# jnbraun/bcnn

Hardware: AMD Instinct MI355X
Metric: images/sec fwd+bwd (higher is better)
Workload: dtype f32; 1 GPU; ResNet-18 224x224 (BASELINE configs[2]), N=128 per GPU, fwd+bwd+SGD through bcnn_net C API; CIFAR-example topology + ImageNet stem, fc-1000; batch_per_gpu=128, global_batch=128, parallelism=dp1, comm=none (one rank)

## Files before the change

### bcnn_amd/csrc/conv_dw_dma.hip

```cpp
#include "conv_paths.h"
#include "lds_dma.h"

namespace bcnn_hip {

struct DwDmaArgs {
    const float* x;
    const float* dy;
    float* partials;
    ConvShape s;
    int mtiles, ntiles;
    int qsplits, q_per_split;
    int Mpad, Npad;
    unsigned x_bytes, dy_bytes;
    unsigned ow_magic;
    int b_row_stride;
    int kk2;
    int rowmode, nrows, row_kk, row_ks, row_plane, row_pitch;
    unsigned row_kk_magic, row_ks_magic;
};

constexpr int DWQ = 32;
constexpr int DWPAIR = 66;

template <int WM, int WN, int WTM, int WTN>
__global__ __launch_bounds__(64 * WM * WN) void conv_dw_dma_kernel(const DwDmaArgs a) {
    constexpr int NW = WM * WN;
    constexpr int BM = 32 * WM * WTM, BN = 32 * WN * WTN;
    static_assert((BM / 2) % NW == 0 && (BN / 2) % NW == 0, "row pairs must split evenly over the waves");
    constexpr int APAIRS = BM / 2, BPAIRS = BN / 2;
    constexpr int BUF = (APAIRS + BPAIRS) * DWPAIR;
    __shared__ float lds[2 * BUF];

    const ConvShape& s = a.s;
    const int tid = threadIdx.x, lane = tid & 63;
    const int wid = __builtin_amdgcn_readfirstlane(tid >> 6);
    const int wm = wid / WN, wn = wid % WN;
    const int l31 = lane & 31, lhi = lane >> 5;
    const int g = blockIdx.y;
    const int lb = xcd_remap(blockIdx.x, gridDim.x);
    const int tap = lb % a.kk2;
    const int rest = lb / a.kk2;
    const int tiles = a.mtiles * a.ntiles;
    const int tile = rest % tiles, qs = rest / tiles;
    const int mt = tile % a.mtiles, nt = tile / a.mtiles;
    const int f0 = mt * BM, c0 = nt * BN;
    const int kr = s.pointwise ? 0 : tap / s.ksz, kc = s.pointwise ? 0 : tap - (tap / s.ksz) * s.ksz;

    const unsigned qbeg = (unsigned)qs * (unsigned)a.q_per_split;
    unsigned qend = qbeg + (unsigned)a.q_per_split;
    if (qend > (unsigned)s.total_q) qend = (unsigned)s.total_q;
    const int nkt = qbeg < qend ? (int)((qend - qbeg + DWQ - 1) / DWQ) : 0;

    unsigned q = qbeg + (unsigned)l31;
    unsigned n = q / (unsigned)s.OHOW;
    unsigned pix = q - n * (unsigned)s.OHOW;
    const unsigned row_a = (unsigned)lhi * (unsigned)s.OHOW, row_b = a.rowmode ? 0u : (unsigned)lhi * (unsigned)a.b_row_stride;
    unsigned va = kOOB, vb = kOOB;
    auto lane_offsets = [&]() {
        const bool qv = q < qend;
        const unsigned offa = n * (unsigned)(s.F * s.OHOW) + pix + row_a;
        unsigned offb;
        bool ok = qv;
        if (s.pointwise) {
            offb = n * (unsigned)(s.C * s.HW) + pix + row_b;
        } else {
            const unsigned oh = magic_div(pix, a.ow_magic), ow = pix - oh * (unsigned)s.OW;
            const int ih = (int)oh * s.stride - s.pad + kr, iw = (int)ow * s.stride - s.pad + kc;
            ok = ok && (unsigned)ih < (unsigned)s.H && (unsigned)iw < (unsigned)s.W;
            offb = (n * (unsigned)(s.C * s.H) + (unsigned)ih) * (unsigned)s.W + (unsigned)iw + row_b;
        }
        va = qv ? offa * 4u : kOOB;
        vb = ok ? offb * 4u : kOOB;
    };
    auto advance = [&]() {
        q += DWQ; pix += DWQ;
        if (pix >= (unsigned)s.OHOW) { pix -= (unsigned)s.OHOW; ++n; }
    };

    const rsrc_i4 rs_a = make_rsrc(a.dy, a.dy_bytes), rs_b = make_rsrc(a.x, a.x_bytes);
    const unsigned lds0 = lds_offset(&lds[0]);
    const unsigned a_row0 = (unsigned)(g * s.Mg), b_grp = (unsigned)(g * s.Cg) * (unsigned)s.HW;

    auto stage = [&](int buf) {
        const unsigned base = lds0 + (unsigned)(buf * BUF * 4);
#pragma unroll
        for (int i = 0; i < APAIRS / NW; ++i) {
            const int p = wid * (APAIRS / NW) + i;
            const int f = f0 + 2 * p;
            const unsigned soff = (a_row0 + (unsigned)(f < s.Mg ? f : 0)) * (unsigned)s.OHOW * 4u;
            dma_row(rs_a, base + (unsigned)(p * DWPAIR * 4), va, soff);
        }
#pragma unroll
        for (int i = 0; i < BPAIRS / NW; ++i) {
            const int p = wid * (BPAIRS / NW) + i;
            const int c = c0 + 2 * p;
            if (a.rowmode) {
                auto row_off = [&](int j) -> unsigned {
                    if (j >= a.nrows) j = 0;
                    const unsigned ch = magic_div((unsigned)j, a.row_kk_magic), r = (unsigned)j - ch * (unsigned)a.row_kk;
                    const unsigned kr = magic_div(r, a.row_ks_magic), kc = r - kr * (unsigned)a.row_ks;
                    return (ch * (unsigned)a.row_plane + kr * (unsigned)a.row_pitch + kc) * 4u;
                };
                const unsigned o0 = row_off(c), o1 = row_off(c + 1);
                const unsigned vbp = vb == kOOB ? kOOB : vb + (unsigned)lhi * (o1 - o0);
                dma_row(rs_b, base + (unsigned)((APAIRS + p) * DWPAIR * 4), vbp, o0);
            } else {
                const unsigned soff = (b_grp + (unsigned)(c < s.Cg ? c : 0) * (unsigned)a.b_row_stride) * 4u;
                dma_row(rs_b, base + (unsigned)((APAIRS + p) * DWPAIR * 4), vb, soff);
            }
        }
    };

    f32x16 acc[WTM][WTN];
#pragma unroll
    for (int i = 0; i < WTM; ++i)
#pragma unroll
        for (int j = 0; j < WTN; ++j)
#pragma unroll
            for (int r = 0; r < 16; ++r) acc[i][j][r] = 0.f;

    int a_off[WTM], b_off[WTN];
#pragma unroll
    for (int i = 0; i < WTM; ++i) a_off[i] = ((wm * WTM + i) * 16 + (l31 >> 1)) * DWPAIR + (l31 & 1) * 32 + 2 * lhi;
#pragma unroll
    for (int j = 0; j < WTN; ++j) b_off[j] = (APAIRS + (wn * WTN + j) * 16 + (l31 >> 1)) * DWPAIR + (l31 & 1) * 32 + 2 * lhi;

    if (nkt > 0) {
        lane_offsets();
        stage(0);
    }
    dma_wait();
    __syncthreads();
    for (int it = 0; it < nkt; ++it) {
        const int cur = it & 1;
        if (it + 1 < nkt) {
            advance();
            lane_offsets();
            stage(cur ^ 1);
        }
        const float* buf = lds + cur * BUF;
#pragma unroll
        for (int kp = 0; kp < DWQ / 4; ++kp) {
            float2 av[WTM], bv[WTN];
#pragma unroll
            for (int i = 0; i < WTM; ++i) av[i] = *reinterpret_cast<const float2*>(buf + a_off[i] + 4 * kp);
#pragma unroll
            for (int j = 0; j < WTN; ++j) bv[j] = *reinterpret_cast<const float2*>(buf + b_off[j] + 4 * kp);
#pragma unroll
            for (int i = 0; i < WTM; ++i)
#pragma unroll
                for (int j = 0; j < WTN; ++j) acc[i][j] = mfma32(av[i].x, bv[j].x, acc[i][j]);
#pragma unroll
            for (int i = 0; i < WTM; ++i)
#pragma unroll
                for (int j = 0; j < WTN; ++j) acc[i][j] = mfma32(av[i].y, bv[j].y, acc[i][j]);
        }
        dma_wait();
        __syncthreads();
    }

    float* out = a.partials + ((((size_t)qs * s.groups + g) * a.kk2 + tap) * a.Mpad) * (size_t)a.Npad;
#pragma unroll
    for (int i = 0; i < WTM; ++i)
#pragma unroll
        for (int j = 0; j < WTN; ++j) {
            float v[16];
#pragma unroll
            for (int r = 0; r < 16; ++r) v[r] = acc[i][j][r];
#pragma unroll
            for (int r = 0; r < 16; ++r) {
                const int f = f0 + (wm * WTM + i) * 32 + mfma_row(r, lane);
                const int c = c0 + (wn * WTN + j) * 32 + l31;
                out[(size_t)f * a.Npad + c] = v[r];
            }
        }
}

template <int NSUB>
__global__ __launch_bounds__(64 * NSUB) void conv_dw_dma_finalize_kernel(const float* __restrict__ partials,
                                                                        int qsplits, int groups, int Mg, int Cg,
                                                                        int kk2, int Mpad, int Npad,
                                                                        float* __restrict__ dw,
                                                                        const float* __restrict__ fold_var,
                                                                        const float* __restrict__ fold_scales) {
    __shared__ float red[NSUB][64];
    const int tx = threadIdx.x & 63, ty = threadIdx.x >> 6;
    const size_t total = (size_t)groups * kk2 * Mg * Cg;
    const size_t i = (size_t)blockIdx.x * 64 + tx;
    const size_t plane = (size_t)Mpad * Npad;
    const size_t qstride = (size_t)groups * kk2 * plane;
    float sum = 0.f;
    size_t o = 0;
    if (i < total) {
        const int c = (int)(i % Cg);
        size_t t = i / Cg;
        const int f = (int)(t % Mg);
        t /= Mg;
        const int tap = (int)(t % kk2), g = (int)(t / kk2);
        const float* p = partials + ((size_t)g * kk2 + tap) * plane + (size_t)f * Npad + c;
        int qs = ty;
        float s0 = 0.f, s1 = 0.f, s2 = 0.f, s3 = 0.f;
        for (; qs + 3 * NSUB < qsplits; qs += 4 * NSUB) {
            const float v0 = p[(size_t)qs * qstride], v1 = p[(size_t)(qs + NSUB) * qstride];
            const float v2 = p[(size_t)(qs + 2 * NSUB) * qstride], v3 = p[(size_t)(qs + 3 * NSUB) * qstride];
            s0 += v0; s1 += v1; s2 += v2; s3 += v3;
        }
        for (; qs < qsplits; qs += NSUB) s0 += p[(size_t)qs * qstride];
        sum = (s0 + s1) + (s2 + s3);
        o = (((size_t)g * Mg + f) * Cg + c) * kk2 + tap;
    }
    red[ty][tx] = sum;
    __syncthreads();
    if (ty == 0 && i < total) {
        float tot = 0.f;
#pragma unroll
        for (int r = 0; r < NSUB; ++r) tot += red[r][tx];
        if (fold_var) tot *= bnfold_a(fold_var, fold_scales, (int)((i / ((size_t)Mg * Cg * kk2)) * Cg + (i % Cg)));
        dw[o] += tot;
    }
}

template <int NSUB>
__global__ __launch_bounds__(64 * NSUB) void conv_dw_dma_finalize_x4_kernel(const float* __restrict__ partials, int qsplits,
                                                                           int groups, int Mg, int Cg, int Mpad, int Npad,
                                                                           float* __restrict__ dw,
                                                                           const float* __restrict__ fold_var,
                                                                           const float* __restrict__ fold_scales) {
    __shared__ float4 red[NSUB][64];
    const int tx = threadIdx.x & 63, ty = threadIdx.x >> 6;
    const size_t total4 = (size_t)groups * Mg * Cg / 4;
    const size_t i4 = (size_t)blockIdx.x * 64 + tx;
    const size_t plane = (size_t)Mpad * Npad;
    const size_t qstride = (size_t)groups * plane;
    float4 sum = make_float4(0.f, 0.f, 0.f, 0.f);
    if (i4 < total4) {
        const size_t i = i4 * 4;
        const int c = (int)(i % Cg);
        const size_t t = i / Cg;
        const int f = (int)(t % Mg), g = (int)(t / Mg);
        const float* p = partials + (size_t)g * plane + (size_t)f * Npad + c;
        auto ld = [&](int qs) { return *reinterpret_cast<const float4*>(p + (size_t)qs * qstride); };
        auto acc = [](float4& a, const float4& v) { a.x += v.x; a.y += v.y; a.z += v.z; a.w += v.w; };
        float4 s0 = sum, s1 = sum, s2 = sum, s3 = sum;
        int qs = ty;
        for (; qs + 3 * NSUB < qsplits; qs += 4 * NSUB) {
            const float4 v0 = ld(qs), v1 = ld(qs + NSUB), v2 = ld(qs + 2 * NSUB), v3 = ld(qs + 3 * NSUB);
            acc(s0, v0); acc(s1, v1); acc(s2, v2); acc(s3, v3);
        }
        for (; qs < qsplits; qs += NSUB) acc(s0, ld(qs));
        sum = make_float4((s0.x + s1.x) + (s2.x + s3.x), (s0.y + s1.y) + (s2.y + s3.y), (s0.z + s1.z) + (s2.z + s3.z),
                          (s0.w + s1.w) + (s2.w + s3.w));
    }
    red[ty][tx] = sum;
    __syncthreads();
    if (ty == 0 && i4 < total4) {
        float4 tot = make_float4(0.f, 0.f, 0.f, 0.f);
#pragma unroll
        for (int r = 0; r < NSUB; ++r) { tot.x += red[r][tx].x; tot.y += red[r][tx].y; tot.z += red[r][tx].z; tot.w += red[r][tx].w; }
        float4* o = reinterpret_cast<float4*>(dw) + i4;
        if (fold_var) {
            const size_t i = i4 * 4;
            const int c = (int)(i % Cg) + (int)(i / ((size_t)Mg * Cg)) * Cg;
            tot.x *= bnfold_a(fold_var, fold_scales, c); tot.y *= bnfold_a(fold_var, fold_scales, c + 1);
            tot.z *= bnfold_a(fold_var, fold_scales, c + 2); tot.w *= bnfold_a(fold_var, fold_scales, c + 3);
        }
        float4 d = *o;
        d.x += tot.x; d.y += tot.y; d.z += tot.z; d.w += tot.w;
        *o = d;
    }
}

struct DwTile { int bm, bn, threads; };
constexpr int kNumDwTiles = 6;
static const DwTile kDwTiles[kNumDwTiles] = {
    {64, 64, 256},
    {128, 64, 256},
    {128, 64, 512},
    {128, 128, 256},
    {128, 128, 1024},
    {64, 128, 512},
};

struct DwDmaPlan {
    bool ok;
    int cfg;
    int mtiles, ntiles, qsplits, q_per_split, Mpad, Npad, kk2;
    size_t partial_floats;
};

static DwDmaPlan plan_dw_dma(const ConvShape& s) {
    DwDmaPlan p;
    p.ok = false;
    p.partial_floats = 0;
    if (s.ksz > 7 && !s.pointwise) return p;
    if (s.Mg < 32 || s.Cg < 16 || (s.Mg & 1) || (s.Cg & 1)) return p;
    if (s.OHOW < DWQ || s.total_q < 4 * DWQ) return p;
    if ((size_t)s.N * s.C * s.HW * 4 >= 0x7ffffff0ull || (size_t)s.N * s.F * s.OHOW * 4 >= 0x7ffffff0ull) return p;
    p.kk2 = s.pointwise ? 1 : s.ksz * s.ksz;
    p.cfg = s.Mg > 64 ? 1 : 0;
    static const char* forced = BCNN_EXP_ENV("BCNN_HIP_DW_TILE");
    if (forced && forced[0] >= '0' && forced[0] < '0' + kNumDwTiles) p.cfg = forced[0] - '0';
    static const char* wantenv = BCNN_EXP_ENV("BCNN_HIP_DW_WANT");
    const int want_per_cu = wantenv ? atoi(wantenv) : 8;
    const int BM = kDwTiles[p.cfg].bm, BN = kDwTiles[p.cfg].bn;
    p.mtiles = ceil_div(s.Mg, BM); p.ntiles = ceil_div(s.Cg, BN);
    p.Mpad = p.mtiles * BM; p.Npad = p.ntiles * BN;
    const long long tiles = (long long)p.mtiles * p.ntiles * p.kk2 * s.groups;
    long long want = ((long long)want_per_cu * kCUs + tiles - 1) / tiles;
    const long long maxs = (s.total_q + 8 * DWQ - 1) / (8 * DWQ);
    if (want > maxs) want = maxs;
    if (want < 1) want = 1;
    long long per = (s.total_q + want - 1) / want;
    per = (per + DWQ - 1) / DWQ * DWQ;
    p.q_per_split = (int)per;
    p.qsplits = (int)((s.total_q + per - 1) / per);
    p.partial_floats = (size_t)p.qsplits * s.groups * p.kk2 * (size_t)p.Mpad * p.Npad;
    p.ok = true;
    return p;
}

size_t conv_dw_dma_workspace_floats(const ConvShape& s) { return plan_dw_dma(s).partial_floats; }


bool conv_backward_weights_dma(const float* x, const float* dy, float* dw, const ConvShape& s, float* workspace,
                               size_t workspace_floats, const BnFold* fold) {
    const DwDmaPlan p = plan_dw_dma(s);
    if (!p.ok) return false;
    conv_require_workspace(workspace, workspace_floats, p.partial_floats);
    DwDmaArgs a;
    a.rowmode = 0; a.nrows = 0;
    a.x = x; a.dy = dy; a.partials = workspace; a.s = s;
    a.mtiles = p.mtiles; a.ntiles = p.ntiles; a.qsplits = p.qsplits; a.q_per_split = p.q_per_split;
    a.Mpad = p.Mpad; a.Npad = p.Npad; a.kk2 = p.kk2;
    a.x_bytes = (unsigned)((size_t)s.N * s.C * s.HW * 4);
    a.dy_bytes = (unsigned)((size_t)s.N * s.F * s.OHOW * 4);
    a.ow_magic = magic_of(s.OW);
    a.b_row_stride = s.pointwise ? s.OHOW : s.HW;
    dim3 grid((unsigned)(p.mtiles * p.ntiles * p.kk2 * p.qsplits), (unsigned)s.groups);
    const unsigned threads = (unsigned)kDwTiles[p.cfg].threads;
    trace_kernel("conv_dw_dma_kernel");
    switch (p.cfg) {
        case 0: conv_dw_dma_kernel<2, 2, 1, 1><<<grid, threads, 0, current_stream()>>>(a); break;
        case 1: conv_dw_dma_kernel<2, 2, 2, 1><<<grid, threads, 0, current_stream()>>>(a); break;
        case 2: conv_dw_dma_kernel<4, 2, 1, 1><<<grid, threads, 0, current_stream()>>>(a); break;
        case 3: conv_dw_dma_kernel<2, 2, 2, 2><<<grid, threads, 0, current_stream()>>>(a); break;
        case 4: conv_dw_dma_kernel<4, 4, 1, 1><<<grid, threads, 0, current_stream()>>>(a); break;
        default: conv_dw_dma_kernel<2, 4, 1, 1><<<grid, threads, 0, current_stream()>>>(a); break;
    }
    KERNEL_CHECK();
    const size_t total = (size_t)s.groups * s.Mg * s.Cg * p.kk2;
    static const bool x4_on = BCNN_EXP_ENV("BCNN_HIP_NO_DW_FINALIZE_X4") == nullptr;
    if (x4_on && p.kk2 == 1 && p.qsplits > 16 && (s.Cg & 3) == 0 && (p.Npad & 3) == 0 &&
        ((reinterpret_cast<uintptr_t>(dw) | reinterpret_cast<uintptr_t>(workspace)) & 15) == 0)
        conv_dw_dma_finalize_x4_kernel<16><<<(unsigned)((total / 4 + 63) / 64), 1024, 0, current_stream()>>>(
            workspace, p.qsplits, s.groups, s.Mg, s.Cg, p.Mpad, p.Npad, dw, fold ? fold->var : nullptr, fold ? fold->scales : nullptr);
    else if (p.qsplits > 16)
        conv_dw_dma_finalize_kernel<16><<<(unsigned)((total + 63) / 64), 1024, 0, current_stream()>>>(
            workspace, p.qsplits, s.groups, s.Mg, s.Cg, p.kk2, p.Mpad, p.Npad, dw, fold ? fold->var : nullptr, fold ? fold->scales : nullptr);
    else
        conv_dw_dma_finalize_kernel<4><<<(unsigned)((total + 63) / 64), 256, 0, current_stream()>>>(
            workspace, p.qsplits, s.groups, s.Mg, s.Cg, p.kk2, p.Mpad, p.Npad, dw, fold ? fold->var : nullptr, fold ? fold->scales : nullptr);
    KERNEL_CHECK();
    return true;
}

bool conv_backward_weights_dma_timed(const float* x, const float* dy, float* dw, float*, const ConvShape& s, float* workspace,
                                     size_t workspace_floats, bool*) {
    if (!plan_dw_dma(s).ok) return false;
    KTimer kt(K_CONV_DW, conv_gemm_flops(s), conv_gemm_bytes(s));
    return conv_backward_weights_dma(x, dy, dw, s, workspace, workspace_floats, nullptr);
}


static DwDmaPlan plan_dw_small_c(const ConvShape& s) {
    DwDmaPlan p;
    p.ok = false; p.partial_floats = 0;
    if (!conv_small_c_fwd_wanted(s) || (s.Mg & 1) || s.OHOW < DWQ || s.total_q < 4 * DWQ) return p;
    p.kk2 = 1;
    p.cfg = 0;
    const int BM = kDwTiles[p.cfg].bm, BN = kDwTiles[p.cfg].bn;
    p.mtiles = ceil_div(s.Mg, BM); p.ntiles = ceil_div(s.K, BN);
    p.Mpad = p.mtiles * BM; p.Npad = p.ntiles * BN;
    const long long tiles = (long long)p.mtiles * p.ntiles;
    long long want = (8LL * kCUs + tiles - 1) / tiles;
    const long long maxs = (s.total_q + 8 * DWQ - 1) / (8 * DWQ);
    if (want > maxs) want = maxs;
    if (want < 1) want = 1;
    long long per = (s.total_q + want - 1) / want;
    per = (per + DWQ - 1) / DWQ * DWQ;
    p.q_per_split = (int)per;
    p.qsplits = (int)((s.total_q + per - 1) / per);
    p.partial_floats = (size_t)p.qsplits * (size_t)p.Mpad * p.Npad;
    p.ok = true;
    return p;
}

size_t conv_dw_small_c_workspace_floats(const ConvShape& s) { return plan_dw_small_c(s).partial_floats; }

bool conv_backward_weights_small_c(const float* x, const float* dy, float* dw, float*, const ConvShape& s, float* workspace,
                                   size_t workspace_floats, bool*) {
    const DwDmaPlan p = plan_dw_small_c(s);
    if (!p.ok) return false;
    conv_require_workspace(workspace, workspace_floats, p.partial_floats);
    KTimer kt(K_CONV_DW, conv_gemm_flops(s), conv_gemm_bytes(s));
    const int Hp = s.H + 2 * s.pad, Wp = s.W + 2 * s.pad;
    float* xp = conv_small_c_padded_input(x, s, 0, nullptr, 1);
    const ConvShape sp = make_conv_shape(s.N, s.C, Hp, Wp, s.F, s.ksz, s.stride, 0, 1);
    DwDmaArgs a;
    a.x = xp; a.dy = dy; a.partials = workspace; a.s = sp;
    a.mtiles = p.mtiles; a.ntiles = p.ntiles; a.qsplits = p.qsplits; a.q_per_split = p.q_per_split;
    a.Mpad = p.Mpad; a.Npad = p.Npad; a.kk2 = 1;
    a.x_bytes = (unsigned)((size_t)s.N * s.C * Hp * Wp * 4);
    a.dy_bytes = (unsigned)((size_t)s.N * s.F * s.OHOW * 4);
    a.ow_magic = magic_of(sp.OW);
    a.b_row_stride = 0;
    a.rowmode = 1; a.nrows = s.K; a.row_kk = s.ksz * s.ksz; a.row_ks = s.ksz; a.row_plane = Hp * Wp; a.row_pitch = Wp;
    a.row_kk_magic = magic_of(a.row_kk); a.row_ks_magic = magic_of(a.row_ks);
    dim3 grid((unsigned)(p.mtiles * p.ntiles * p.qsplits), 1u);
    conv_dw_dma_kernel<2, 2, 1, 1><<<grid, (unsigned)kDwTiles[0].threads, 0, current_stream()>>>(a);
    KERNEL_CHECK();
    const size_t total = (size_t)s.Mg * s.K;
    if (p.qsplits > 16)
        conv_dw_dma_finalize_kernel<16><<<(unsigned)((total + 63) / 64), 1024, 0, current_stream()>>>(
            workspace, p.qsplits, 1, s.Mg, s.K, 1, p.Mpad, p.Npad, dw, nullptr, nullptr);
    else
        conv_dw_dma_finalize_kernel<4><<<(unsigned)((total + 63) / 64), 256, 0, current_stream()>>>(
            workspace, p.qsplits, 1, s.Mg, s.K, 1, p.Mpad, p.Npad, dw, nullptr, nullptr);
    KERNEL_CHECK();
    return true;
}

}
```

### bcnn_amd/csrc/conv_winograd_fused.hip

```cpp
#include "conv_paths.h"
#include "lds_dma.h"
#include "wino43_pack.h"

namespace bcnn_hip {

constexpr int WF_BT = 64;
constexpr int WF_BF = 64;
constexpr int WF_KC = 8;
constexpr int WF_STAGE = 16 * WF_KC * (WF_BF + WF_BT);

struct WinoFusedArgs {
    const float* src;
    const float* upk;
    float* dst;
    const float* bias;
    const float* slopes;
    float* stats;
    int N, J, M, H, W, TH, TW;
    unsigned T;
    int Jpad, Mpad, mblocks, tblocks;
    int nfull;
    int nunits;
    int act, add_bias;
    unsigned src_bytes, upk_bytes, dst_bytes, stats_bytes;
// ... 460 lines not shown
    const unsigned grid = (unsigned)(nblocks < kCUs ? nblocks : kCUs);
    const int rem = nblocks % (int)grid;
    a.nfull = (rem > 0 && 2 * rem <= (int)grid && nblocks > (int)grid) ? nblocks - rem : nblocks;
    a.nunits = a.nfull + 2 * (nblocks - a.nfull);
    const bool plain = !a.add_bias && a.act == BCNN_HIP_ACT_NONE;
    a.tail_scr = nullptr; a.tail_q = 0; a.tail_units = 0; a.tail_scr_bytes = 0;
    static const int ksplit_on = BCNN_EXP_ENV("BCNN_HIP_NO_WINO_KSPLIT") ? 0 : 1;
    if (ksplit_on && plain && !parts && rem > 0 && nblocks > (int)grid) {
        const int NC = a.Jpad / WF_KC;
        const int q = (int)ceil_div((long long)rem * NC, (long long)grid);
        const double ep = 1.5, now = (a.nfull < nblocks ? 0.5 * NC : (double)NC) + ep, split = q + 2 * ep + 2.0;
        if (q >= 1 && q <= NC && split < now) {
            a.nfull = nblocks;
            a.nunits = nblocks - rem;
            a.tail_units = rem;
            a.tail_q = q;
            const size_t scr_floats = (size_t)2 * grid * 64 * 64 * 4;
            a.tail_scr = scratch(SCRATCH_WFUSED_TAIL, scr_floats);
            a.tail_scr_bytes = (unsigned)(scr_floats * sizeof(float));
        }
    }
    a.stats_bytes = a.stats ? (unsigned)((size_t)a.M * 2 * a.tblocks * 2 * sizeof(float)) : 0u;
    if (a.stats && (size_t)a.stats_bytes > stats->capacity * sizeof(float)) {
        fprintf(stderr, "[bcnn_hip] fused Winograd: statistics need %u bytes, the caller's buffer holds %zu\n",
                a.stats_bytes, stats->capacity * sizeof(float));
        abort();
    }
    if (a.stats && !plain) {
        fprintf(stderr, "[bcnn_hip] fused Winograd: output statistics are taken on the raw convolution output only\n");
        abort();
    }
    trace_kernel(dx_mode ? "wino_fused_kernel:dx" : "wino_fused_kernel:fwd");
#ifdef BCNN_HIP_EXPERIMENT
    if (parts == 2) { wino_bf16_launch<2>(a, w, s, dx_mode, grid, plain); }
    else if (parts == 3) { wino_bf16_launch<3>(a, w, s, dx_mode, grid, plain); }
    else
#endif
    if (a.stats) wino_fused_kernel<0, true><<<grid, 512, 0, current_stream()>>>(a);
    else if (plain) wino_fused_kernel<0, false><<<grid, 512, 0, current_stream()>>>(a);
    else if (a.act == BCNN_HIP_ACT_RELU) wino_fused_kernel<1, false><<<grid, 512, 0, current_stream()>>>(a);
    else wino_fused_kernel<2, false><<<grid, 512, 0, current_stream()>>>(a);
    KERNEL_CHECK();
    if (a.tail_units > 0) {
        trace_kernel("wino_tail_fixup");
        if (a.stats) wino_tail_fixup_kernel<true><<<(unsigned)(a.tail_units * 16), 256, 0, current_stream()>>>(a);
        else wino_tail_fixup_kernel<false><<<(unsigned)(a.tail_units * 16), 256, 0, current_stream()>>>(a);
        KERNEL_CHECK();
    }
    if (stats) stats->splits = a.stats ? 2 * a.tblocks : 0;
}

bool wino_fused_pack_plan(const ConvShape& s, int dx_mode, WinoPackJob* job, size_t* floats) {
    const int J = dx_mode ? s.F : s.C, M = dx_mode ? s.C : s.F;
    if (wino_bf16_parts(J) != 0) return false;
    job->w = nullptr; job->u = nullptr;
    job->F = s.F; job->C = s.C; job->dx_mode = dx_mode;
    job->Jpad = (J + WF_KC - 1) / WF_KC * WF_KC;
    job->Mpad = (M + WF_BF - 1) / WF_BF * WF_BF;
    job->blocks = (int)ceil_div((long long)job->Jpad * job->Mpad, 256);
    job->npos = 16;
    job->layout = 0;
    *floats = (size_t)16 * job->Jpad * job->Mpad;
    return true;
}

void wino_fused_pack_launch(const WinoPackJob* jobs_dev, int n, int max_blocks) {
    wino_pack_weights_multi_kernel<<<dim3((unsigned)max_blocks, (unsigned)n), 256, 0, current_stream()>>>(jobs_dev);
    KERNEL_CHECK();
}

static double wf_flops(const ConvShape& s) {
    const double T = (double)s.N * ((s.H + 1) / 2) * ((s.W + 1) / 2);
    return 2.0 * 16.0 * T * s.C * s.F;
}
static double wf_useful_flops(const ConvShape& s) { return 2.0 * 16.0 * ((double)s.N * s.H * s.W / 4.0) * s.C * s.F; }

bool conv_winograd_fused_fwd_wanted(const ConvShape& s, int) { return wino_fused_wanted(s, s.C, s.F); }
void conv_forward_winograd_fused(const ConvFwdCall& c) {
    const ConvShape& s = c.s;
    KTimer kt(K_CONV_FWD_WINO, wf_flops(s), conv_gemm_bytes(s), wf_useful_flops(s));
    wino_fused_run(c.x, c.w, c.y, s, 0, c.bias, c.slopes, c.raw ? BCNN_HIP_ACT_NONE : c.act, c.raw ? 0 : (c.bias != nullptr),
                   c.raw ? c.stats : nullptr);
}

bool conv_winograd_fused_dx_wanted(const ConvShape& s, int) { return wino_fused_wanted(s, s.F, s.C); }
void conv_backward_data_winograd_fused(const ConvDxCall& c) {
    const ConvShape& s = c.s;
    KTimer kt(K_CONV_DX_WINO, wf_flops(s), conv_gemm_bytes(s), wf_useful_flops(s));
    wino_fused_run(c.dy, c.w, c.dx, s, 1, nullptr, nullptr, BCNN_HIP_ACT_NONE, 0, nullptr);
}


constexpr int WD_KT = 8;
constexpr int WD_ROW = WD_KT;
constexpr int WD_OP = 16 * 64 * WD_ROW;


struct WinoDwArgs {
    const float* x;
    const float* dy;
    float* partials;
    int N, C, F, H, W, TH, TW;
    unsigned T, tiles_per_split;
    int fblocks, cblocks, splits;
    unsigned x_bytes, dy_bytes;
};

template <bool ODDW>
__global__ __launch_bounds__(512, 2) void wino_dw_fused_kernel(const WinoDwArgs a) {
    __shared__ __attribute__((aligned(16))) float lds[2 * 2 * WD_OP];
    const int tid = threadIdx.x, lane = tid & 63;
    const int wid = __builtin_amdgcn_readfirstlane(tid >> 6);
    const int l31 = lane & 31, lhi = lane >> 5;
    const int nob = a.fblocks * a.cblocks;
    const int ob = blockIdx.x % nob, sp = blockIdx.x / nob;
    const int f0 = (ob % a.fblocks) * 64, c0 = (ob / a.fblocks) * 64;
    const unsigned tbeg = (unsigned)sp * a.tiles_per_split;
    unsigned tend = tbeg + a.tiles_per_split;
    if (tend > a.T) tend = a.T;
    const int nchunks = tbeg < tend ? (int)((tend - tbeg + WD_KT - 1) / WD_KT) : 0;

    const int tl = lane & 7, ch = wid * 8 + (lane >> 3);
    const bool f_ok = f0 + ch < a.F, c_ok = c0 + ch < a.C;
    const bool is_l = tl == 0, is_r = tl == 7;
    unsigned t = tbeg + (unsigned)tl;
    const unsigned per_img = (unsigned)(a.TH * a.TW);
    int th, tw;
    unsigned xo, yo;
    {
        const int n = (int)(t / per_img);
        const unsigned rr = t - (unsigned)n * per_img;
        th = (int)(rr / (unsigned)a.TW);
        tw = (int)(rr - (unsigned)th * (unsigned)a.TW);
        xo = (unsigned)(((n * a.C + c0 + ch) * a.H + 2 * th) * a.W + 2 * tw) * 4u;
        yo = (unsigned)(((n * a.F + f0 + ch) * a.H + 2 * th) * a.W + 2 * tw) * 4u;
    }
    const unsigned W4 = (unsigned)a.W * 4u;
    const unsigned step_row = (unsigned)(2 * a.W - 2 * a.TW) * 4u;
    const unsigned step_img_x = (unsigned)(a.C * a.H * a.W - 2 * a.W * a.TH) * 4u;
    const unsigned step_img_y = (unsigned)(a.F * a.H * a.W - 2 * a.W * a.TH) * 4u;
    const rsrc_i4 rs_x = make_rsrc(a.x, a.x_bytes), rs_y = make_rsrc(a.dy, a.dy_bytes);

    constexpr bool odd_w = ODDW;
    buf_f32x2 xm[4], gy[2];
    float xl[4], xr[4];
    bool sel_l = false, sel_r = false, pair_y_ok = true;
    auto load_items = [&]() {
        const bool live = t < tend;
        const bool x_ok = live && c_ok, y_ok = live && f_ok;
        const bool r0 = th > 0, r2 = 2 * th + 1 < a.H, r3 = 2 * th + 2 < a.H;
        const bool has_l = tw > 0, has_r = tw + 1 < a.TW;
        sel_l = !is_l && has_l;
        sel_r = !is_r && has_r;
        if (odd_w) pair_y_ok = 2 * tw + 1 < a.W;
        const bool el = x_ok && is_l && has_l, er = x_ok && is_r && has_r;
        const unsigned up = xo - W4;
        const int s1 = __builtin_amdgcn_readfirstlane((int)W4), s2 = __builtin_amdgcn_readfirstlane((int)(2u * W4));
        xm[0] = buffer_load_f32x2(rs_x, (int)((x_ok && r0) ? up : kOOB), 0, 0);
        xm[1] = buffer_load_f32x2(rs_x, (int)(x_ok ? xo : kOOB), 0, 0);
        xm[2] = buffer_load_f32x2(rs_x, (int)((x_ok && r2) ? xo : kOOB), s1, 0);
        xm[3] = buffer_load_f32x2(rs_x, (int)((x_ok && r3) ? xo : kOOB), s2, 0);
        xl[0] = buffer_load_f32(rs_x, (int)((el && r0) ? up - 4u : kOOB), 0, 0);
        xl[1] = buffer_load_f32(rs_x, (int)(el ? xo - 4u : kOOB), 0, 0);
        xl[2] = buffer_load_f32(rs_x, (int)((el && r2) ? xo - 4u : kOOB), s1, 0);
        xl[3] = buffer_load_f32(rs_x, (int)((el && r3) ? xo - 4u : kOOB), s2, 0);
        xr[0] = buffer_load_f32(rs_x, (int)((er && r0) ? up + 8u : kOOB), 0, 0);
        xr[1] = buffer_load_f32(rs_x, (int)(er ? xo + 8u : kOOB), 0, 0);
        xr[2] = buffer_load_f32(rs_x, (int)((er && r2) ? xo + 8u : kOOB), s1, 0);
        xr[3] = buffer_load_f32(rs_x, (int)((er && r3) ? xo + 8u : kOOB), s2, 0);
        gy[0] = buffer_load_f32x2(rs_y, (int)(y_ok ? yo : kOOB), 0, 0);
        gy[1] = buffer_load_f32x2(rs_y, (int)((y_ok && r2) ? yo : kOOB), s1, 0);
    };
    auto advance = [&]() {
        t += WD_KT;
        tw += WD_KT;
        const bool c1 = tw >= a.TW, c2 = tw >= 2 * a.TW;
        const int rows = (c1 ? 1 : 0) + (c2 ? 1 : 0);
        tw -= rows * a.TW;
        th += rows;
        const bool ci = th >= a.TH;
        if (ci) th -= a.TH;
        const unsigned d = 64u + (c1 ? step_row : 0u) + (c2 ? step_row : 0u);
        xo += d + (ci ? step_img_x : 0u);
        yo += d + (ci ? step_img_y : 0u);
    };
    float d[4][4], g[2][2];
    auto assemble = [&]() {
#pragma unroll
        for (int i = 0; i < 4; ++i) {
            float m0 = xm[i][0], m1 = xm[i][1];
            if (odd_w) m1 = pair_y_ok ? m1 : 0.f;
            const float fromleft = __builtin_bit_cast(float, __builtin_amdgcn_mov_dpp(__builtin_bit_cast(int, m1), 0x111 , 0xf, 0xf, true));
            const float fromright = __builtin_bit_cast(float, __builtin_amdgcn_mov_dpp(__builtin_bit_cast(int, m0), 0x101 , 0xf, 0xf, true));
            d[i][0] = sel_l ? fromleft : xl[i];
            d[i][1] = m0;
            d[i][2] = m1;
            d[i][3] = sel_r ? fromright : xr[i];
        }
#pragma unroll
        for (int r = 0; r < 2; ++r) {
            g[r][0] = gy[r][0];
            g[r][1] = odd_w ? (pair_y_ok ? gy[r][1] : 0.f) : gy[r][1];
        }
    };
    auto write_items = [&](int stage) {
        assemble();
        float* pm = lds + stage * 2 * WD_OP + ch * WD_ROW + (tl ^ (2 * (wid & 3) + lhi));
        float* pv = pm + WD_OP;
        float q[4][2];
#pragma unroll
        for (int c = 0; c < 2; ++c) {
            q[0][c] = g[0][c];
            q[1][c] = g[0][c] + g[1][c];
            q[2][c] = g[0][c] - g[1][c];
            q[3][c] = -g[1][c];
        }
#pragma unroll
        for (int i = 0; i < 4; ++i) {
            pm[(4 * i + 0) * 64 * WD_ROW] = q[i][0];
            pm[(4 * i + 1) * 64 * WD_ROW] = q[i][0] + q[i][1];
            pm[(4 * i + 2) * 64 * WD_ROW] = q[i][0] - q[i][1];
            pm[(4 * i + 3) * 64 * WD_ROW] = -q[i][1];
        }
        float tt[4][4];
#pragma unroll
        for (int j = 0; j < 4; ++j) {
            tt[0][j] = d[0][j] - d[2][j];
            tt[1][j] = d[1][j] + d[2][j];
            tt[2][j] = d[2][j] - d[1][j];
            tt[3][j] = d[1][j] - d[3][j];
        }
#pragma unroll
        for (int i = 0; i < 4; ++i) {
            pv[(4 * i + 0) * 64 * WD_ROW] = tt[i][0] - tt[i][2];
            pv[(4 * i + 1) * 64 * WD_ROW] = tt[i][1] + tt[i][2];
            pv[(4 * i + 2) * 64 * WD_ROW] = tt[i][2] - tt[i][1];
            pv[(4 * i + 3) * 64 * WD_ROW] = tt[i][1] - tt[i][3];
        }
    };

    f32x16 acc[2][2][2];
#pragma unroll
    for (int e = 0; e < 2; ++e)
#pragma unroll
        for (int i = 0; i < 2; ++i)
#pragma unroll
            for (int j = 0; j < 2; ++j)
#pragma unroll
                for (int r = 0; r < 16; ++r) acc[e][i][j][r] = 0.f;

    const bool early = wid < 4;
    const unsigned rd0 = (unsigned)(((2 * wid) * 64 + l31) * WD_ROW + (lhi ^ ((l31 >> 2) & 1)) + 2 * ((l31 >> 3) & 3));
    if (nchunks > 0) {
        load_items();
        write_items(0);
        if (nchunks > 1) {
            advance();
            load_items();
        }
    }
    __syncthreads();
    for (int kc = 0; kc < nchunks; ++kc) {
        const int cur = kc & 1, nxt = cur ^ 1;
        const bool more = kc + 1 < nchunks, more2 = kc + 2 < nchunks;
        auto produce = [&]() {
            if (more) write_items(nxt);
            if (more2) {
                advance();
                load_items();
            }
        };
        if (early) produce();
        __builtin_amdgcn_sched_barrier(0);
        const float* stage_base = lds + cur * 2 * WD_OP;
#pragma unroll
        for (int ks = 0; ks < WD_KT / 2; ++ks) {
            float af[2][2], bf[2][2];
            const float* ms = stage_base + (rd0 ^ (unsigned)(2 * ks));
            const float* vs = ms + WD_OP;
#pragma unroll
            for (int e = 0; e < 2; ++e)
#pragma unroll
                for (int i = 0; i < 2; ++i) {
                    af[e][i] = ms[(e * 64 + i * 32) * WD_ROW];
                    bf[e][i] = vs[(e * 64 + i * 32) * WD_ROW];
                }
#pragma unroll
            for (int e = 0; e < 2; ++e)
#pragma unroll
                for (int i = 0; i < 2; ++i)
#pragma unroll
                    for (int j = 0; j < 2; ++j) {
                        acc[e][i][j] = mfma32(af[e][i], bf[e][j], acc[e][i][j]);
                    }
            if (ks == WD_KT / 4 - 1 && !early) {
                __builtin_amdgcn_sched_barrier(0);
                produce();
                __builtin_amdgcn_sched_barrier(0);
            }
        }
        __builtin_amdgcn_sched_barrier(0);
        __syncthreads();
    }
    float* out = a.partials + ((size_t)sp * nob + ob) * (size_t)(16 * 64 * 64);
#pragma unroll
    for (int e = 0; e < 2; ++e)
#pragma unroll
        for (int i = 0; i < 2; ++i)
#pragma unroll
            for (int j = 0; j < 2; ++j)
#pragma unroll
                for (int r = 0; r < 16; ++r)
                    out[((2 * wid + e) * 64 + i * 32 + mfma_row(r, lane)) * 64 + j * 32 + l31] = acc[e][i][j][r];
}

__global__ __launch_bounds__(256) void wino_dw_fused_finalize_kernel(const float* __restrict__ partials, int splits,
                                                                     int fblocks, int cblocks, int F, int C,
                                                                     float* __restrict__ dw) {
    __shared__ float u[16][65];
    const int xi = threadIdx.x >> 4, cq = threadIdx.x & 15;
    const int nob = fblocks * cblocks;
    const int fl = blockIdx.x & 63, ob = blockIdx.x >> 6;
    const float* p = partials + (size_t)ob * (16 * 64 * 64) + ((size_t)xi * 64 + fl) * 64 + cq * 4;
    const size_t stride = (size_t)nob * (16 * 64 * 64);
    float4 s0 = make_float4(0.f, 0.f, 0.f, 0.f), s1 = s0, s2 = s0, s3 = s0;
    auto ld = [&](int sp) { return *reinterpret_cast<const float4*>(p + (size_t)sp * stride); };
    auto add = [](float4& s, const float4& v) { s.x += v.x; s.y += v.y; s.z += v.z; s.w += v.w; };
    int sp = 0;
    for (; sp + 3 < splits; sp += 4) {
        const float4 v0 = ld(sp), v1 = ld(sp + 1), v2 = ld(sp + 2), v3 = ld(sp + 3);
        add(s0, v0); add(s1, v1); add(s2, v2); add(s3, v3);
    }
    for (; sp < splits; ++sp) add(s0, ld(sp));
    u[xi][cq * 4 + 0] = (s0.x + s1.x) + (s2.x + s3.x);
    u[xi][cq * 4 + 1] = (s0.y + s1.y) + (s2.y + s3.y);
    u[xi][cq * 4 + 2] = (s0.z + s1.z) + (s2.z + s3.z);
    u[xi][cq * 4 + 3] = (s0.w + s1.w) + (s2.w + s3.w);
    __syncthreads();
    const int q = threadIdx.x;
    const int f = (ob % fblocks) * 64 + fl, c = (ob / fblocks) * 64 + q;
    if (q < 64 && f < F && c < C) {
        float m[4][4];
#pragma unroll
        for (int k = 0; k < 16; ++k) m[k >> 2][k & 3] = u[k][q];
        float t[3][4];
#pragma unroll
        for (int j = 0; j < 4; ++j) {
            t[0][j] = m[0][j] + 0.5f * (m[1][j] + m[2][j]);
            t[1][j] = 0.5f * (m[1][j] - m[2][j]);
            t[2][j] = 0.5f * (m[1][j] + m[2][j]) + m[3][j];
        }
        float* o = dw + ((size_t)f * C + c) * 9;
#pragma unroll
        for (int r = 0; r < 3; ++r) {
            o[r * 3 + 0] += t[r][0] + 0.5f * (t[r][1] + t[r][2]);
            o[r * 3 + 1] += 0.5f * (t[r][1] - t[r][2]);
            o[r * 3 + 2] += 0.5f * (t[r][1] + t[r][2]) + t[r][3];
        }
    }
}

struct WinoDwPlan {
    bool ok;
    int fblocks, cblocks, splits;
    unsigned T, tiles_per_split;
    size_t partial_floats;
};

static int g_wd_force = -1;
static WinoDwPlan wino_dw_fused_plan(const ConvShape& s, int cus = kCUs) {
    WinoDwPlan p;
    p.ok = false; p.partial_floats = 0;
    if (s.ksz != 3 || s.stride != 1 || s.pad != 1 || s.groups != 1) return p;
    const int TW = (s.W + 1) / 2, TH = (s.H + 1) / 2;
    if (TW < 4 || TH < 2 || s.C < 32 || s.F < 32) return p;
    if ((size_t)s.N * s.C * s.HW * 4 >= 0x7ffffff0ull || (size_t)s.N * s.F * s.HW * 4 >= 0x7ffffff0ull) return p;
    if (g_wd_force < 0) {
        const char* e = BCNN_EXP_ENV("BCNN_HIP_WINOGRAD_DW_FUSED");
        g_wd_force = e ? (e[0] == '0' ? 0 : 1) : 2;
    }
    if (g_wd_force == 0) return p;
    if (g_wd_force == 2 && (s.C < 64 || s.F < 64)) return p;
    p.T = (unsigned)((long long)s.N * TH * TW);
    p.fblocks = (s.F + 63) / 64; p.cblocks = (s.C + 63) / 64;
    const int nob = p.fblocks * p.cblocks;
    static const char* const dw_cus_str = BCNN_EXP_ENV("BCNN_HIP_DW_CUS");
    static const int dw_cus_env = dw_cus_str ? atoi(dw_cus_str) : 0;
    int splits = (dw_cus_env > 0 ? dw_cus_env : cus) / nob;
    if (splits < 1) splits = 1;
    unsigned per = (p.T + (unsigned)splits - 1) / (unsigned)splits;
    per = (per + WD_KT - 1) / WD_KT * WD_KT;
    if (per < 4 * WD_KT) per = 4 * WD_KT;
    p.tiles_per_split = per;
    p.splits = (int)((p.T + per - 1) / per);
    if (g_wd_force == 2 && p.splits * nob < cus / 2) return p;
    p.partial_floats = (size_t)p.splits * nob * (16 * 64 * 64);
    p.ok = true;
    return p;
}

size_t conv_dw_winograd_fused_workspace_floats(const ConvShape& s) { return wino_dw_fused_plan(s).partial_floats; }

bool conv_backward_weights_winograd_fused(const float* x, const float* dy, float* dw, float*, const ConvShape& s,
                                          float* workspace, size_t workspace_floats, bool*) {
    const bool yield_cus = conv_side_stream_deferred() && s.HW >= 784 && wino_dw_fused_plan(s).ok;
    const WinoDwPlan p = wino_dw_fused_plan(s, yield_cus ? kCUs * 3 / 4 : kCUs);
    if (!p.ok) return false;
    if (reinterpret_cast<uintptr_t>(workspace) & 15) return false;
    conv_require_workspace(workspace, workspace_floats, p.partial_floats);
    KTimer kt(K_CONV_DW_WINO, wf_flops(s), conv_gemm_bytes(s), wf_useful_flops(s));
    WinoDwArgs a;
    a.x = x; a.dy = dy; a.partials = workspace;
    a.N = s.N; a.C = s.C; a.F = s.F; a.H = s.H; a.W = s.W; a.TH = (s.H + 1) / 2; a.TW = (s.W + 1) / 2;
    a.T = p.T; a.tiles_per_split = p.tiles_per_split;
    a.fblocks = p.fblocks; a.cblocks = p.cblocks; a.splits = p.splits;
    a.x_bytes = (unsigned)((size_t)s.N * s.C * s.HW * 4);
    a.dy_bytes = (unsigned)((size_t)s.N * s.F * s.HW * 4);
    const int nob = p.fblocks * p.cblocks;
    trace_kernel("wino_dw_fused_kernel");
    if (s.W & 1) wino_dw_fused_kernel<true><<<(unsigned)(p.splits * nob), 512, 0, current_stream()>>>(a);
    else wino_dw_fused_kernel<false><<<(unsigned)(p.splits * nob), 512, 0, current_stream()>>>(a);
    KERNEL_CHECK();
    wino_dw_fused_finalize_kernel<<<(unsigned)(nob * 64), 256, 0, current_stream()>>>(workspace, p.splits, p.fblocks, p.cblocks,
                                                                                      s.F, s.C, dw);
    KERNEL_CHECK();
    return true;
}

}
```

Baseline: 13900 images/s.

## Apply Winograd output transform in dW kernel; vectorize tap-major dW finalize

The fused Winograd weight-gradient kernel now stages its accumulators through LDS and applies the 4x4-to-3x3 inverse transform before writing partials. Each split therefore stores 9 taps instead of 16, which shrinks the partial workspace and the finalize kernel's reads. The finalize kernel then only sums 9 taps per split and writes contiguous dw rows with coalesced adds. Separately, the DMA dW path gains a float4 split-reduction finalize kernel for 3x3 (kk2==9) weights. The cost is extra LDS traffic and synchronization in the main kernel's epilogue.

```diff
diff --git a/bcnn_amd/csrc/conv_dw_dma.hip b/bcnn_amd/csrc/conv_dw_dma.hip
--- a/bcnn_amd/csrc/conv_dw_dma.hip
+++ b/bcnn_amd/csrc/conv_dw_dma.hip
@@ -267,6 +267,60 @@
         float4 d = *o;
         d.x += tot.x; d.y += tot.y; d.z += tot.z; d.w += tot.w;
         *o = d;
+    }
+}
+
+template <int NSUB>
+__global__ __launch_bounds__(64 * NSUB) void conv_dw_dma_finalize_taps_x4_kernel(const float* __restrict__ partials, int qsplits,
+                                                                                int groups, int Mg, int Cg, int kk2, int Mpad,
+                                                                                int Npad, float* __restrict__ dw,
+                                                                                const float* __restrict__ fold_var,
+                                                                                const float* __restrict__ fold_scales) {
+    __shared__ float4 red[NSUB][64];
+    const int tx = threadIdx.x & 63, ty = threadIdx.x >> 6;
+    const size_t total4 = (size_t)groups * kk2 * Mg * Cg / 4;
+    const size_t i4 = (size_t)blockIdx.x * 64 + tx;
+    const size_t plane = (size_t)Mpad * Npad;
+    const size_t qstride = (size_t)groups * kk2 * plane;
+    float4 sum = make_float4(0.f, 0.f, 0.f, 0.f);
+    size_t o = 0;
+    int cg = 0;
+    if (i4 < total4) {
+        const size_t i = i4 * 4;
+        const int c = (int)(i % Cg);
+        size_t t = i / Cg;
+        const int f = (int)(t % Mg);
+        t /= Mg;
+        const int tap = (int)(t % kk2), g = (int)(t / kk2);
+        const float* p = partials + ((size_t)g * kk2 + tap) * plane + (size_t)f * Npad + c;
+        auto ld = [&](int qs) { return *reinterpret_cast<const float4*>(p + (size_t)qs * qstride); };
+        auto acc = [](float4& a, const float4& v) { a.x += v.x; a.y += v.y; a.z += v.z; a.w += v.w; };
+        float4 s0 = sum, s1 = sum, s2 = sum, s3 = sum;
+        int qs = ty;
+        for (; qs + 3 * NSUB < qsplits; qs += 4 * NSUB) {
+            const float4 v0 = ld(qs), v1 = ld(qs + NSUB), v2 = ld(qs + 2 * NSUB), v3 = ld(qs + 3 * NSUB);
+            acc(s0, v0); acc(s1, v1); acc(s2, v2); acc(s3, v3);
+        }
+        for (; qs < qsplits; qs += NSUB) acc(s0, ld(qs));
+        sum = make_float4((s0.x + s1.x) + (s2.x + s3.x), (s0.y + s1.y) + (s2.y + s3.y), (s0.z + s1.z) + (s2.z + s3.z),
+                          (s0.w + s1.w) + (s2.w + s3.w));
+        o = (((size_t)g * Mg + f) * Cg + c) * kk2 + tap;
+        cg = g * Cg + c;
+    }
+    red[ty][tx] = sum;
+    __syncthreads();
+    if (ty == 0 && i4 < total4) {
+        float4 tot = make_float4(0.f, 0.f, 0.f, 0.f);
+#pragma unroll
+        for (int r = 0; r < NSUB; ++r) { tot.x += red[r][tx].x; tot.y += red[r][tx].y; tot.z += red[r][tx].z; tot.w += red[r][tx].w; }
+        if (fold_var) {
+            tot.x *= bnfold_a(fold_var, fold_scales, cg); tot.y *= bnfold_a(fold_var, fold_scales, cg + 1);
+            tot.z *= bnfold_a(fold_var, fold_scales, cg + 2); tot.w *= bnfold_a(fold_var, fold_scales, cg + 3);
+        }
+        dw[o] += tot.x;
+        dw[o + kk2] += tot.y;
+        dw[o + 2 * (size_t)kk2] += tot.z;
+        dw[o + 3 * (size_t)kk2] += tot.w;
     }
 }
 
@@ -354,7 +408,14 @@
         ((reinterpret_cast<uintptr_t>(dw) | reinterpret_cast<uintptr_t>(workspace)) & 15) == 0)
         conv_dw_dma_finalize_x4_kernel<16><<<(unsigned)((total / 4 + 63) / 64), 1024, 0, current_stream()>>>(
             workspace, p.qsplits, s.groups, s.Mg, s.Cg, p.Mpad, p.Npad, dw, fold ? fold->var : nullptr, fold ? fold->scales : nullptr);
-    else if (p.qsplits > 16)
+    else if (x4_on && p.kk2 == 9 && (s.Cg & 3) == 0 && (p.Npad & 3) == 0 && (reinterpret_cast<uintptr_t>(workspace) & 15) == 0) {
+        if (p.qsplits > 16)
+            conv_dw_dma_finalize_taps_x4_kernel<16><<<(unsigned)((total / 4 + 63) / 64), 1024, 0, current_stream()>>>(
+                workspace, p.qsplits, s.groups, s.Mg, s.Cg, p.kk2, p.Mpad, p.Npad, dw, fold ? fold->var : nullptr, fold ? fold->scales : nullptr);
+        else
+            conv_dw_dma_finalize_taps_x4_kernel<4><<<(unsigned)((total / 4 + 63) / 64), 256, 0, current_stream()>>>(
+                workspace, p.qsplits, s.groups, s.Mg, s.Cg, p.kk2, p.Mpad, p.Npad, dw, fold ? fold->var : nullptr, fold ? fold->scales : nullptr);
+    } else if (p.qsplits > 16)
         conv_dw_dma_finalize_kernel<16><<<(unsigned)((total + 63) / 64), 1024, 0, current_stream()>>>(
             workspace, p.qsplits, s.groups, s.Mg, s.Cg, p.kk2, p.Mpad, p.Npad, dw, fold ? fold->var : nullptr, fold ? fold->scales : nullptr);
     else
diff --git a/bcnn_amd/csrc/conv_winograd_fused.hip b/bcnn_amd/csrc/conv_winograd_fused.hip
--- a/bcnn_amd/csrc/conv_winograd_fused.hip
+++ b/bcnn_amd/csrc/conv_winograd_fused.hip
@@ -786,62 +786,79 @@
         __builtin_amdgcn_sched_barrier(0);
         __syncthreads();
     }
-    float* out = a.partials + ((size_t)sp * nob + ob) * (size_t)(16 * 64 * 64);
-#pragma unroll
-    for (int e = 0; e < 2; ++e)
-#pragma unroll
-        for (int i = 0; i < 2; ++i)
+    float* out = a.partials + ((size_t)sp * nob + ob) * (size_t)(9 * 64 * 64);
+    const int efl = tid >> 4, ecq = tid & 15;
+#pragma unroll
+    for (int h = 0; h < 2; ++h) {
+        if (h) __syncthreads();
+#pragma unroll
+        for (int e = 0; e < 2; ++e)
 #pragma unroll
             for (int j = 0; j < 2; ++j)
 #pragma unroll
                 for (int r = 0; r < 16; ++r)
-                    out[((2 * wid + e) * 64 + i * 32 + mfma_row(r, lane)) * 64 + j * 32 + l31] = acc[e][i][j][r];
-}
-
-__global__ __launch_bounds__(256) void wino_dw_fused_finalize_kernel(const float* __restrict__ partials, int splits,
+                    lds[((2 * wid + e) * 32 + mfma_row(r, lane)) * 64 + j * 32 + l31] = acc[e][h][j][r];
+        __syncthreads();
+        float4 m[4][4];
+#pragma unroll
+        for (int k = 0; k < 16; ++k) m[k >> 2][k & 3] = *reinterpret_cast<const float4*>(lds + (k * 32 + efl) * 64 + ecq * 4);
+        float4 tr[3][4];
+        auto comb = [](const float4& p, const float4& q, const float4& r, const float4& s, float4& o0, float4& o1, float4& o2) {
+            o0 = make_float4(p.x + 0.5f * (q.x + r.x), p.y + 0.5f * (q.y + r.y), p.z + 0.5f * (q.z + r.z), p.w + 0.5f * (q.w + r.w));
+            o1 = make_float4(0.5f * (q.x - r.x), 0.5f * (q.y - r.y), 0.5f * (q.z - r.z), 0.5f * (q.w - r.w));
+            o2 = make_float4(0.5f * (q.x + r.x) + s.x, 0.5f * (q.y + r.y) + s.y, 0.5f * (q.z + r.z) + s.z, 0.5f * (q.w + r.w) + s.w);
+        };
+#pragma unroll
+        for (int j = 0; j < 4; ++j) comb(m[0][j], m[1][j], m[2][j], m[3][j], tr[0][j], tr[1][j], tr[2][j]);
+        float* o = out + (h * 32 + efl) * 64 + ecq * 4;
+#pragma unroll
+        for (int r = 0; r < 3; ++r) {
+            float4 o0, o1, o2;
+            comb(tr[r][0], tr[r][1], tr[r][2], tr[r][3], o0, o1, o2);
+            *reinterpret_cast<float4*>(o + (r * 3 + 0) * 64 * 64) = o0;
+            *reinterpret_cast<float4*>(o + (r * 3 + 1) * 64 * 64) = o1;
+            *reinterpret_cast<float4*>(o + (r * 3 + 2) * 64 * 64) = o2;
+        }
+    }
+}
+
+__global__ __launch_bounds__(192) void wino_dw_fused_finalize_kernel(const float* __restrict__ partials, int splits,
                                                                      int fblocks, int cblocks, int F, int C,
                                                                      float* __restrict__ dw) {
-    __shared__ float u[16][65];
-    const int xi = threadIdx.x >> 4, cq = threadIdx.x & 15;
+    __shared__ float u[64 * 9];
     const int nob = fblocks * cblocks;
     const int fl = blockIdx.x & 63, ob = blockIdx.x >> 6;
-    const float* p = partials + (size_t)ob * (16 * 64 * 64) + ((size_t)xi * 64 + fl) * 64 + cq * 4;
-    const size_t stride = (size_t)nob * (16 * 64 * 64);
-    float4 s0 = make_float4(0.f, 0.f, 0.f, 0.f), s1 = s0, s2 = s0, s3 = s0;
-    auto ld = [&](int sp) { return *reinterpret_cast<const float4*>(p + (size_t)sp * stride); };
-    auto add = [](float4& s, const float4& v) { s.x += v.x; s.y += v.y; s.z += v.z; s.w += v.w; };
-    int sp = 0;
-    for (; sp + 3 < splits; sp += 4) {
-        const float4 v0 = ld(sp), v1 = ld(sp + 1), v2 = ld(sp + 2), v3 = ld(sp + 3);
-        add(s0, v0); add(s1, v1); add(s2, v2); add(s3, v3);
-    }
-    for (; sp < splits; ++sp) add(s0, ld(sp));
-    u[xi][cq * 4 + 0] = (s0.x + s1.x) + (s2.x + s3.x);
-    u[xi][cq * 4 + 1] = (s0.y + s1.y) + (s2.y + s3.y);
-    u[xi][cq * 4 + 2] = (s0.z + s1.z) + (s2.z + s3.z);
-    u[xi][cq * 4 + 3] = (s0.w + s1.w) + (s2.w + s3.w);
+    const int tap = threadIdx.x >> 4, cq = threadIdx.x & 15;
+    if (tap < 9) {
+        const float* p = partials + (size_t)ob * (9 * 64 * 64) + ((size_t)tap * 64 + fl) * 64 + cq * 4;
+        const size_t stride = (size_t)nob * (9 * 64 * 64);
+        float4 s = make_float4(0.f, 0.f, 0.f, 0.f);
+        auto ld = [&](int sp) { return *reinterpret_cast<const float4*>(p + (size_t)sp * stride); };
+        auto add = [](float4& s, const float4& v) { s.x += v.x; s.y += v.y; s.z += v.z; s.w += v.w; };
+        int sp = 0;
+        for (; sp + 7 < splits; sp += 8) {
+            float4 v[8];
+#pragma unroll
+            for (int k = 0; k < 8; ++k) v[k] = ld(sp + k);
+#pragma unroll
+            for (int k = 0; k < 8; ++k) add(s, v[k]);
+        }
+        for (; sp + 3 < splits; sp += 4) {
+            const float4 v0 = ld(sp), v1 = ld(sp + 1), v2 = ld(sp + 2), v3 = ld(sp + 3);
+            add(s, v0); add(s, v1); add(s, v2); add(s, v3);
+        }
+        for (; sp < splits; ++sp) add(s, ld(sp));
+        u[(cq * 4 + 0) * 9 + tap] = s.x;
+        u[(cq * 4 + 1) * 9 + tap] = s.y;
+        u[(cq * 4 + 2) * 9 + tap] = s.z;
+        u[(cq * 4 + 3) * 9 + tap] = s.w;
+    }
     __syncthreads();
-    const int q = threadIdx.x;
-    const int f = (ob % fblocks) * 64 + fl, c = (ob / fblocks) * 64 + q;
-    if (q < 64 && f < F && c < C) {
-        float m[4][4];
-#pragma unroll
-        for (int k = 0; k < 16; ++k) m[k >> 2][k & 3] = u[k][q];
-        float t[3][4];
-#pragma unroll
-        for (int j = 0; j < 4; ++j) {
-            t[0][j] = m[0][j] + 0.5f * (m[1][j] + m[2][j]);
-            t[1][j] = 0.5f * (m[1][j] - m[2][j]);
-            t[2][j] = 0.5f * (m[1][j] + m[2][j]) + m[3][j];
-        }
-        float* o = dw + ((size_t)f * C + c) * 9;
-#pragma unroll
-        for (int r = 0; r < 3; ++r) {
-            o[r * 3 + 0] += t[r][0] + 0.5f * (t[r][1] + t[r][2]);
-            o[r * 3 + 1] += 0.5f * (t[r][1] - t[r][2]);
-            o[r * 3 + 2] += 0.5f * (t[r][1] + t[r][2]) + t[r][3];
-        }
-    }
+    const int f = (ob % fblocks) * 64 + fl, c0 = (ob / fblocks) * 64;
+    if (f >= F) return;
+    const int live = (C - c0 < 64 ? C - c0 : 64) * 9;
+    float* o = dw + ((size_t)f * C + c0) * 9;
+    for (int j = threadIdx.x; j < live; j += 192) o[j] += u[j];
 }
 
 struct WinoDwPlan {
@@ -878,7 +895,7 @@
     p.tiles_per_split = per;
     p.splits = (int)((p.T + per - 1) / per);
     if (g_wd_force == 2 && p.splits * nob < cus / 2) return p;
-    p.partial_floats = (size_t)p.splits * nob * (16 * 64 * 64);
+    p.partial_floats = (size_t)p.splits * nob * (9 * 64 * 64);
     p.ok = true;
     return p;
 }
@@ -905,7 +922,7 @@
     if (s.W & 1) wino_dw_fused_kernel<true><<<(unsigned)(p.splits * nob), 512, 0, current_stream()>>>(a);
     else wino_dw_fused_kernel<false><<<(unsigned)(p.splits * nob), 512, 0, current_stream()>>>(a);
     KERNEL_CHECK();
-    wino_dw_fused_finalize_kernel<<<(unsigned)(nob * 64), 256, 0, current_stream()>>>(workspace, p.splits, p.fblocks, p.cblocks,
+    wino_dw_fused_finalize_kernel<<<(unsigned)(nob * 64), 192, 0, current_stream()>>>(workspace, p.splits, p.fblocks, p.cblocks,
                                                                                       s.F, s.C, dw);
     KERNEL_CHECK();
     return true;
```

Result: no change. 13990 images/s, median of 6 (+0.6%).
